# l13039968960/stm32H7-YOLO

Measured on AMD Instinct MI355X. Metric: images/sec int8 YOLO-face 56x56, higher is better.
Workload: dtype int8; 1 GPU; BASELINE configs[1]: batch=4096 int8 YOLO-face 56x56x3 frames per GPU, fused LDS-resident forward + GPU box decode; frames_per_gpu=4096, global_batch=4096, frame_bytes_in=9408, frame_bytes_out=882, input_batches_rotated=8, input_bytes_resident=308281344, kernel=yoloface56_fused<F=2,NW=8>, requant_rounding=ref, parallelism=single GPU, gather_every=1, collectives_issued=0, launch_streams=2

## Files before the change

### stm32h7-yolo_amd/csrc/yf_fused56.hip.h

```cpp


template <class B, int C, int F, int NT>
__device__ __forceinline__ void dump_buf(const char* frames, int8_t* dump, long stride, long off, long first_frame,
                                         long n_frames, int tid, int ch0 = 0, int split = 1 << 30, int gap = 0) {
  if (!dump) return;
  for (int i = tid; i < F * B::P * C; i += NT) {
    const int ch = i % C; const int t = i / C;
    const int p = t % B::P; const int f = t / B::P;
    if (first_frame + f >= n_frames) continue;
    const int phys = ch0 + ch + (ch >= split ? gap : 0);
    dump[(first_frame + f) * stride + off + (long)p * C + ch] = (int8_t)frames[f * B::FS + B::at_p(p) + phys];
  }
}

template <class B, int C, int FT, int NT, class IdOf>
__device__ __forceinline__ void dump_sets(const char* frames, int8_t* dump, long stride, long off, const IdOf& id_of, int tid, int ch0 = 0, int split = 1 << 30, int gap = 0) {
  for (int i = tid; i < FT * B::P * C; i += NT) {
    const int ch = i % C; const int t = i / C;
    const int p = t % B::P; const int f = t / B::P;
    const long id = id_of(f);
    if (id < 0) continue;
    const int phys = ch0 + ch + (ch >= split ? gap : 0);
    dump[id * stride + off + (long)p * C + ch] = (int8_t)frames[f * B::FS + B::at_p(p) + phys];
  }
}

struct DumpOffsets {
  enum { T1 = 0, T2 = T1 + 6272, T3 = T2 + 6272, T4 = T3 + 3136, Q21 = T4 + 14112, T6 = Q21 + 3528, T7 = T6 + 3528,
         T8 = T7 + 1176, T9 = T8 + 7056, T11 = T9 + 7056, T14 = T11 + 1176, T15 = T14 + 7056, Q45 = T15 + 4704,
         T17 = Q45 + 1176, T18 = T17 + 1176, T19 = T18 + 392, T20 = T19 + 1960, T22 = T20 + 1960, T23 = T22 + 392,
         T24 = T23 + 1960, T26 = T24 + 1960, T30 = T26 + 392, T31 = T30 + 2352, T32 = T31 + 1960, T33 = T32 + 1960,
         P8 = T33 + 1568, C17 = P8 + 3528, P25 = C17 + 1176, C34 = P25 + 1176, C40 = C34 + 392, L43 = C40 + 392,
         TOTAL = L43 + 1176 };
};

struct NetParams {
  const int8_t* in;
  int8_t* out;
  long n;
  const uint8_t* tab;
  int8_t* dump;
  int stop_stage;
  yf_det* dets;
  int* counts;
  int cap, mode;
  int q_thr;
  float w_scale, h_scale;
  char* scratch;
};
static_assert(sizeof(yf_table_index) <= YF_INDEX_RESERVED, "index does not fit its reserved slot");
typedef const __attribute__((address_space(4))) char* kargs_ptr;
__device__ __forceinline__ kargs_ptr kargs_here() {
  kargs_ptr p = (kargs_ptr)__builtin_amdgcn_kernarg_segment_ptr();
  asm volatile("" : "+s"(p));
  return p;
}
#define YF_ARG(FIELD) (*reinterpret_cast<const __attribute__((address_space(4))) decltype(NetParams::FIELD)*>(kargs_here() + offsetof(NetParams, FIELD)))

#ifndef YF_POOL_MERGE
#define YF_POOL_MERGE 1
#endif
#ifndef YF_POOL8H_WAVES
#define YF_POOL8H_WAVES 3
#endif
#ifndef YF_POOL8V_WAVES
#define YF_POOL8V_WAVES 3
#endif
#ifndef YF_PRIO_LIST
#define YF_PRIO_LIST 3,3,3,3,3,3,3,3,3,3, 2,2,2,2, 1,1,1,1,1,1, 0,0,0,0,0,0,0
#endif
constexpr int STAGE_PRIO[27] = {YF_PRIO_LIST};
template <int K> __device__ __forceinline__ void stage_prio() {
  if constexpr (K == 0 || STAGE_PRIO[K] != STAGE_PRIO[K - 1]) __builtin_amdgcn_s_setprio(STAGE_PRIO[K]);
}
#if defined(YF_LAB) && defined(YF_DUMP_PROD_ORDER)
#define YF_PDUMP 1
#else
#define YF_PDUMP 0
#endif
template <bool DUMP> constexpr bool tail_batch() { return !DUMP || YF_PDUMP; }

template <int F, int NW, bool DUMP, bool CAM = false>
#if !defined(YF_LAB) || !defined(YF_TPJ13)
#undef YF_TPJ13
#define YF_TPJ13 3
#endif
#if !defined(YF_LAB) || !defined(YF_TPJ23)
#undef YF_TPJ23
#define YF_TPJ23 2
#endif
#if defined(YF_LAB) && defined(YF_WHATIF_WPE)
#define YF_WPE(NW) YF_WHATIF_WPE
#else
#define YF_WPE(NW) ((NW) == 12 ? 6 : (NW) >= 8 ? 4 : ((NW) == 6 ? 3 : 2))
#endif
__global__ void __launch_bounds__(NW * 64, YF_WPE(NW)) yoloface56_fused(const NetParams prm) {
  extern __shared__ __attribute__((aligned(16))) char smem[];
  constexpr int NT = NW * 64;
  constexpr bool BATCH = tail_batch<DUMP>();
  constexpr bool POOL_MERGE = YF_POOL_MERGE != 0 && (!DUMP || YF_PDUMP) && NW >= 8;
  constexpr bool XDUMP = DUMP && !YF_PDUMP;
  typedef Buf<B_T14::OFF, 14, 14, 32, 14, 0, 0> B_T6X;
  typedef typename std::conditional<POOL_MERGE, B_T6X, B_T6>::type B_T6M;
  constexpr int FT = BATCH ? 2 * F : F;
  typedef TailBufs<BATCH ? FRAME_STRIDE / 2 : FRAME_STRIDE> U;
  constexpr int OUT_ALL_BYTES = BATCH ? 0 : (F * OUT_FRAME_BYTES + 15) & ~15;
  static_assert(std::is_same<decltype(&yoloface56_fused<F, NW, DUMP, CAM>), void (*)(const NetParams)>::value, "YF_ARG: NetParams is the kernel's only argument (kernarg offset 0)");
  uint8_t* luts = reinterpret_cast<uint8_t*>(smem);
  constexpr int PRE = v2::pre_bytes<F, tail_batch<DUMP>()>();
  char* out_all = smem + PRE;
  char* frames = smem + PRE + OUT_ALL_BYTES;
  const int n_frames = (int)prm.n;
  const int tid0 = threadIdx.x;
  const uint8_t* __restrict__ tab = prm.tab;
  int vz = 0;
  asm volatile("" : "+v"(vz));
  const __attribute__((address_space(1))) uint8_t* lut_src = (const __attribute__((address_space(1))) uint8_t*)(tab + PLAN.lut_off);
  asm volatile("" : "+s"(lut_src));
  for (int i = tid0; i < v2::LUT_B / 16; i += NT)
    reinterpret_cast<v4u*>(luts)[i] = *(const __attribute__((address_space(1))) v4u*)(lut_src + (uint32_t)(16 * i));
  for (int i = tid0; i < v2::ZERO_B / 16; i += NT) reinterpret_cast<uint4*>(smem + v2::ZERO)[i] = uint4{0, 0, 0, 0};
  constexpr int DBG_LUT = PRE + OUT_ALL_BYTES + FRAME_BYTES + (F - 1) * FRAME_STRIDE;
  if constexpr (DUMP) { if (tid0 < YF_DBG_LUT_BYTES / 16) reinterpret_cast<v4u*>(smem + DBG_LUT)[tid0] = *(const __attribute__((address_space(1))) v4u*)(lut_src + (uint32_t)(YF_N_LUT * 256 + YF_ADDLUT_BYTES + 16 * tid0)); }
#if !(defined(YF_LAB) && defined(YF_WHATIF_NO_PROLOGUE_TABLES))
  {
    typedef v2::JobTabs<F, tail_batch<DUMP>()> JTS;
    typedef typename JTS::U UT;
    v2::fill_jobtab<F, 1, B_T1, B_T2, JTS::JT_DW3>(smem, tid0);
    v2::fill_jobtab<F, 2, B_T4, B_T6M, JTS::JT_DW10>(smem, tid0);
    v2::fill_jobtab<F, 1, B_T8, B_T9, JTS::JT_DW15>(smem, tid0);
    v2::fill_jobtab<JTS::FT, 2, typename UT::T15, typename UT::T17, JTS::JT_DW27>(smem, tid0);
    v2::fill_jobtab<JTS::FT, 1, typename UT::T19, typename UT::T20, JTS::JT_DW32>(smem, tid0);
    typedef v2::HaloTabs<F, tail_batch<DUMP>()> HTS;
    v2::build_halotab<typename HTS::G1, HTS::H_T1, NT>(smem, tid0);
    v2::build_halotab<typename HTS::G4, HTS::H_T4, NT>(smem, tid0);
    v2::build_halotab<typename HTS::G8, HTS::H_T8, NT>(smem, tid0);
    v2::build_halotab<typename HTS::G15, HTS::H_T15, NT>(smem, tid0);
    v2::build_halotab<typename HTS::G19, HTS::H_T19, NT>(smem, tid0);
  }
#endif

  auto sfresh = [](int v) { asm volatile("" : "+s"(v)); return v; };
  auto n_groups = [&]() { return (int)((uint32_t)(sfresh(n_frames) + F - 1) / (uint32_t)F); };
  int gstep = (int)gridDim.x;
  asm volatile("" : "+s"(gstep));
  auto park_slot = [&]() { return YF_ARG(scratch) + (uint32_t)(sfresh((int)blockIdx.x) * (F * TailBufs<FRAME_BYTES>::T15_BYTES)); };
  const AddK no_add = {};
  auto addctx = [&](int k) {
    const uint8_t* a = tab + offsetof(yf_table_index, add) + k * sizeof(yf_add);
    return AddK{uniform_u32(a + offsetof(yf_add, mo2)), uniform_u32(a + offsetof(yf_add, zro)),
                (unsigned long)uniform_u32(a + offsetof(yf_add, c64o)) | ((unsigned long)uniform_u32(a + offsetof(yf_add, c64o) + 4) << 32),
                (int)uniform_u32(a + offsetof(yf_add, rso))};
  };
  constexpr long DS = DumpOffsets::TOTAL;
#ifdef YF_BARPROF
  bool prof_on = false;
  int bar_no = 0;
  long long* prof_out = reinterpret_cast<long long*>(prm.dump) + ((long)blockIdx.x * NW + __builtin_amdgcn_readfirstlane(tid0 >> 6)) * 80;
#define YF_SYNC() do { asm volatile("s_waitcnt vmcnt(0)" ::: "memory");    \
                       if (prof_on && (tid0 & 63) == 0 && bar_no < 40) prof_out[2 * bar_no] = __builtin_readcyclecounter(); __syncthreads(); \
                       if (prof_on && (tid0 & 63) == 0 && bar_no < 40) prof_out[2 * bar_no + 1] = __builtin_readcyclecounter(); ++bar_no; } while (0)
#else
#define YF_SYNC() do { asm volatile("s_waitcnt vmcnt(0)" ::: "memory"); __syncthreads(); } while (0)
#endif
#define YF_HALO(B, RING, FR, G, HOFF, WI, TID) \
  do { int ht_ = TID; asm volatile("" : "+v"(ht_)); \
       v2::fill_halo_t<B, typename v2::HaloTabs<F, BATCH>::G, v2::HaloTabs<F, BATCH>::HOFF>(frames, load_halo_zp(tab, WI), ht_); } while (0)
#define YF_FETCH(CS, WV, LN) v2::fetch_consts_s<CS>(tab, WV, LN)
#define YF_CONV1(WV, LN, CS) v2::conv1_2_stage<F, NW, CS>(frames, tab, WV, LN)
#define YF_DENSE(FR, TPJ, KS, BW, IN, OUT, CH0, COUT, EPI, LUT, ADDB, DI, AD, WV, LN, CS) \
  v2::dense2_stage<FR, NW, TPJ, KS, BW, IN, OUT, CH0, COUT, EPI, LUT, ADDB, CS>(frames, out_all, tab, AD, WV, LN)
#define YF_DW(FR, STRIDE, IN, OUT, C, LUT, WI, WV, LN, CS, JTOFF) v2::dw2_stage<FR, NW, STRIDE, IN, OUT, C, LUT, CS, v2::JobTabs<F, BATCH>::JTOFF>(frames, tab, WV, LN)
#define YF_DUMP(BUF, C, OFF, ...) \
  if constexpr (DUMP) { if (prm.dump) { dump_buf<BUF, C, F, NT>(frames, prm.dump, DS, DumpOffsets::OFF, first, n_frames, tid, ##__VA_ARGS__); YF_SYNC(); } }
  int stage_no = 0;
#define YF_STAGE_END() if constexpr (DUMP) { if (++stage_no == prm.stop_stage) continue; }
#define YF_PRIO(K) stage_prio<K>()

  int prev_first = -1;
  auto decode_prev = [&](int w, int ln) {
    if (prm.dets != nullptr && prev_first >= 0 && w >= NW - F && prev_first + (w - (NW - F)) < n_frames) {
      int dl = ln;
      asm volatile("" : "+v"(dl));
      yfdec::decode_frame(reinterpret_cast<const int8_t*>(out_all) + (w - (NW - F)) * OUT_FRAME_BYTES, prev_first + (w - (NW - F)), dl,
                          prm.mode, prm.w_scale, prm.h_scale, prm.dets, prm.counts, prm.cap);
// ... 325 lines not shown
```

### stm32h7-yolo_amd/csrc/yf_kernels.hip.h

```cpp
#include <hip/hip_runtime.h>
#include <stddef.h>
#include <stdint.h>
#include <type_traits>
#include "yf_tables.h"

#pragma clang diagnostic push
#pragma clang diagnostic ignored "-Wint-to-pointer-cast"
#if !defined(YF_LAB) || !defined(YF_LAUNDER)
#undef YF_LAUNDER
#define YF_LAUNDER 0
#endif
#define YF_ROW_SKEW 4
#define YF_T8_ROW_SKEW 32
namespace YF_NS {

#ifndef YF_NOINLINE_STAGES
#define YF_STAGE_FN __device__ __forceinline__
#else
#define YF_STAGE_FN __device__ __attribute__((noinline))
#endif

typedef int v4i __attribute__((ext_vector_type(4)));
typedef short v2s __attribute__((ext_vector_type(2)));

#if !defined(YF_H0) || YF_H0 == 56
constexpr int FRAME_BYTES = 34176;
#endif
constexpr int LUT_BYTES = YF_N_LUT * 256 + YF_ADDLUT_BYTES;


#if !defined(YF_H0) || YF_H0 == 56
#if defined(YF_LAB) && defined(YF_WHATIF_FS)
constexpr int FRAME_STRIDE = YF_WHATIF_FS;
#else
constexpr int FRAME_STRIDE = FRAME_BYTES;
#endif
constexpr int BUF_FS = FRAME_STRIDE;
#else
constexpr int BUF_FS = 0;
#endif
template <int OFF_, int W_, int H_, int S_, int RS_, int PT_, int PL_, int FS_ = BUF_FS, int SK_ = 0>
struct Buf {
  static constexpr int OFF = OFF_, W = W_, H = H_, S = S_, RS = RS_, PT = PT_, PL = PL_, FS = FS_, SK = SK_;
  static constexpr int P = W_ * H_, ROWB = RS_ * S_ + SK_;
  __device__ static __forceinline__ int at(int y, int x) { return OFF_ + (y + PT_) * ROWB + (x + PL_) * S_; }
  __device__ static __forceinline__ int at_p(int p) {
    if constexpr (RS_ == W_ && PT_ == 0 && PL_ == 0) return OFF_ + p * S_;
    else { const int y = p / W_; return at(y, p - y * W_); }
  }
};
template <int WIDTH>
constexpr bool lds_conflict_free(const int (&addr)[32]) {
  for (int i = 0; i < 32; ++i) {
    if (addr[i] % WIDTH != 0) return false;
    for (int j = 0; j < i; ++j)
      if (addr[i] != addr[j] && (addr[i] / WIDTH) % 32 == (addr[j] / WIDTH) % 32) return false;
  }
  return true;
}

#ifndef YF_H0
#define YF_H0 56
#endif
constexpr int G0 = YF_H0, G1 = G0 / 2, G2 = G0 / 4, G3 = G0 / 8;
static_assert(G0 % 8 == 0 && G3 >= 4, "input size must be a multiple of 8 and at least 32");

#if YF_H0 == 56
typedef Buf<    0, 56, 56,  4, 60, 1, 4> B_IN;
typedef Buf<13696, 28, 28,  8, 30, 1, 1, BUF_FS, YF_ROW_SKEW> B_T1;
typedef Buf<21024, 28, 28,  8, 28, 0, 0> B_T2;
typedef Buf<16832, 28, 28,  4, 28, 0, 0> B_T3;
typedef Buf<    0, 28, 28, 20, 29, 1, 1> B_T4;
typedef Buf<16832, 14, 28, 20, 14, 0, 0> B_HB;
typedef Buf<24672, 14, 14, 48, 14, 0, 0> B_T14;
typedef Buf<16832, 14, 14, 32, 14, 0, 0> B_T6;
typedef Buf<    0, 14, 14,  8, 14, 0, 0> B_T7;
typedef Buf< 1568, 14, 14, 36, 16, 1, 1, BUF_FS, YF_T8_ROW_SKEW> B_T8;
typedef Buf<11296, 14, 14, 48, 14, 0, 0> B_T9;
typedef Buf<20704, 14, 14,  8, 14, 0, 0> B_T11;
typedef Buf<    0, 14, 14, 24, 15, 1, 1> B_T15;
typedef Buf< 5408,  7,  7, 48,  7, 0, 0> B_T30;
typedef Buf< 7760,  7,  7, 32,  7, 0, 0> B_T17;
typedef Buf< 9328,  7,  7,  8,  7, 0, 0> B_T18;
typedef Buf< 9728,  7,  7, 40,  9, 1, 1, BUF_FS, YF_ROW_SKEW> B_T19;
typedef Buf<13008,  7,  7, 48,  7, 0, 0> B_T20;
typedef Buf<15360,  7,  7,  8,  7, 0, 0> B_T22;
typedef Buf<15752,  7,  7,  8,  7, 0, 0> B_T26;
typedef Buf<16144,  7,  7, 32,  7, 0, 0> B_T33;
template <int FS_>
struct TailBufs {
  typedef Buf<    0, 14, 14, 24, 15, 1, 1, FS_> T15;
  typedef Buf< 5408,  7,  7, 48,  7, 0, 0, FS_> T30;
  typedef Buf< 7760,  7,  7, 32,  7, 0, 0, FS_> T17;
  typedef Buf< 9328,  7,  7,  8,  7, 0, 0, FS_> T18;
  typedef Buf< 9728,  7,  7, 40,  9, 1, 1, FS_, YF_ROW_SKEW> T19;
  typedef Buf<13008,  7,  7, 48,  7, 0, 0, FS_> T20;
  typedef Buf<15360,  7,  7,  8,  7, 0, 0, FS_> T22;
  typedef Buf<15752,  7,  7,  8,  7, 0, 0, FS_> T26;
  typedef Buf< 7760,  7,  7, 32,  7, 0, 0, FS_> T33;
  typedef Buf<16160,  7,  7, 18,  7, 0, 0, FS_> HEAD;
  static constexpr int END = 16160 + 882, T15_BYTES = 5408;
  static_assert(T19::OFF + 9 * T19::ROWB <= T20::OFF && T20::OFF + 49 * 48 <= T22::OFF && T26::OFF + 49 * 8 <= HEAD::OFF, "tail buffers do not overlap");
#if !(defined(YF_LAB) && defined(YF_WHATIF_FS))
  static_assert(END <= FS_, "a set fits its stride");
#endif
};
#else
constexpr int arena_next(int off, int bytes) { return (off + bytes + 64 + 63) & ~63; }
#define YF_SEQ(NAME, PREV_END, W_, H_, S_, RS_, PT_, PL_, ROWS_)                      \
  constexpr int NAME##_OFF = PREV_END;                                                \
  typedef Buf<NAME##_OFF, W_, H_, S_, RS_, PT_, PL_> NAME;                            \
  constexpr int NAME##_END = arena_next(NAME##_OFF, (ROWS_) * (RS_) * (S_));
YF_SEQ(B_IN,  0,         G0, G0,  4, G0 + 4, 1, 4, G0 + 1)
YF_SEQ(B_T1,  B_IN_END,  G1, G1,  8, G1 + 2, 1, 1, G1 + 2)
YF_SEQ(B_T2,  B_T1_END,  G1, G1,  8, G1,     0, 0, G1)
YF_SEQ(B_T3,  B_T2_END,  G1, G1,  4, G1,     0, 0, G1)
YF_SEQ(B_T4,  B_T3_END,  G1, G1, 20, G1 + 1, 1, 1, G1 + 1)
YF_SEQ(B_HB,  B_T4_END,  G2, G1, 20, G2,     0, 0, G1)
YF_SEQ(B_T14, B_HB_END,  G2, G2, 48, G2,     0, 0, G2)
YF_SEQ(B_T6,  B_T14_END, G2, G2, 32, G2,     0, 0, G2)
YF_SEQ(B_T7,  B_T6_END,  G2, G2,  8, G2,     0, 0, G2)
YF_SEQ(B_T8,  B_T7_END,  G2, G2, 36, G2 + 2, 1, 1, G2 + 2)
YF_SEQ(B_T9,  B_T8_END,  G2, G2, 48, G2,     0, 0, G2)
YF_SEQ(B_T11, B_T9_END,  G2, G2,  8, G2,     0, 0, G2)
YF_SEQ(B_T15, B_T11_END, G2, G2, 24, G2 + 1, 1, 1, G2 + 1)
YF_SEQ(B_T30, B_T15_END, G3, G3, 48, G3,     0, 0, G3)
YF_SEQ(B_T17, B_T30_END, G3, G3, 32, G3,     0, 0, G3)
YF_SEQ(B_T18, B_T17_END, G3, G3,  8, G3,     0, 0, G3)
YF_SEQ(B_T19, B_T18_END, G3, G3, 40, G3 + 2, 1, 1, G3 + 2)
YF_SEQ(B_T20, B_T19_END, G3, G3, 48, G3,     0, 0, G3)
YF_SEQ(B_T22, B_T20_END, G3, G3,  8, G3,     0, 0, G3)
YF_SEQ(B_T26, B_T22_END, G3, G3,  8, G3,     0, 0, G3)
YF_SEQ(B_T33, B_T26_END, G3, G3, 32, G3,     0, 0, G3)
#undef YF_SEQ
#endif

#if YF_H0 != 56
constexpr int FRAME_BYTES = B_T33_END;
#endif
constexpr int OUT_FRAME_BYTES = G3 * G3 * 18;
constexpr int IN_FRAME_BYTES = G0 * G0 * 3;

enum { EPI_LUT = 0, EPI_RAW = 1, EPI_ADD = 2, EPI_HEAD = 3, EPI_HEAD_LDS = 4 };

typedef unsigned v4u __attribute__((ext_vector_type(4)));
typedef unsigned v2u __attribute__((ext_vector_type(2)));
typedef unsigned long v4ul __attribute__((ext_vector_type(4)));
template <bool AFTER_MFMA, bool SIGNLESS = false>
__device__ __forceinline__ void rq4(const v4i acc, const v4u m2, const v4u zr, const v4ul c64, int (&t)[4]) {
  v2u d0, d1, d2, d3;
  if constexpr (SIGNLESS) {
    (void)zr;
#define YF_RQ3_MADS "v_mad_u64_u32 %0, vcc, %4, %8, %12\n\tv_mad_u64_u32 %1, vcc, %5, %9, %13\n\t" \
                    "v_mad_u64_u32 %2, vcc, %6, %10, %14\n\tv_mad_u64_u32 %3, vcc, %7, %11, %15"
#define YF_RQ3_OPS : "=&v"(d0), "=&v"(d1), "=&v"(d2), "=&v"(d3) \
                   : "v"(acc[0]), "v"(acc[1]), "v"(acc[2]), "v"(acc[3]), "v"(m2[0]), "v"(m2[1]), "v"(m2[2]), "v"(m2[3]), \
                     "s"(c64[0]), "s"(c64[1]), "s"(c64[2]), "s"(c64[3]) : "vcc"
    if constexpr (AFTER_MFMA) asm("s_nop 7\n\ts_nop 1\n\t" YF_RQ3_MADS YF_RQ3_OPS);
    else asm(YF_RQ3_MADS YF_RQ3_OPS);
#undef YF_RQ3_MADS
#undef YF_RQ3_OPS
    t[0] = (int)d0[1]; t[1] = (int)d1[1]; t[2] = (int)d2[1]; t[3] = (int)d3[1];
    return;
  }
  unsigned long cy0, cy1, cy2, cy3;
#define YF_RQ4_MADS "v_mad_u64_u32 %0, %4, %8, %12, %16\n\tv_mad_u64_u32 %1, %5, %9, %13, %17\n\t" \
                    "v_mad_u64_u32 %2, %6, %10, %14, %18\n\tv_mad_u64_u32 %3, %7, %11, %15, %19"
#define YF_RQ4_OPS : "=&v"(d0), "=&v"(d1), "=&v"(d2), "=&v"(d3), "=&s"(cy0), "=&s"(cy1), "=&s"(cy2), "=&s"(cy3) \
                   : "v"(acc[0]), "v"(acc[1]), "v"(acc[2]), "v"(acc[3]), "v"(m2[0]), "v"(m2[1]), "v"(m2[2]), "v"(m2[3]), \
                     "s"(c64[0]), "s"(c64[1]), "s"(c64[2]), "s"(c64[3])
  if constexpr (AFTER_MFMA) asm("s_nop 7\n\ts_nop 1\n\t" YF_RQ4_MADS YF_RQ4_OPS);
  else asm(YF_RQ4_MADS YF_RQ4_OPS);
#undef YF_RQ4_MADS
#undef YF_RQ4_OPS
  asm("v_addc_co_u32_e64 %0, vcc, %4, %8, %12\n\tv_addc_co_u32_e64 %1, vcc, %5, %9, %13\n\t"
      "v_addc_co_u32_e64 %2, vcc, %6, %10, %14\n\tv_addc_co_u32_e64 %3, vcc, %7, %11, %15"
      : "=&v"(t[0]), "=&v"(t[1]), "=&v"(t[2]), "=&v"(t[3])
      : "v"(zr[0]), "v"(zr[1]), "v"(zr[2]), "v"(zr[3]), "v"(d0[1]), "v"(d1[1]), "v"(d2[1]), "v"(d3[1]),
        "s"(cy0), "s"(cy1), "s"(cy2), "s"(cy3)
      : "vcc");
}
__device__ __forceinline__ int rqf(int acc, uint32_t fs, int k) {
  const float p = (float)acc * __uint_as_float(fs);
  return min(max(__float_as_int(p + 0x1.8p23f) - k, 0), 255);
}
// ... 449 lines not shown
  }
}

template <int W, int SH = (W > 32 ? 20 : 16)> struct DivW {
  static constexpr uint32_t M = ((1u << SH) + W - 1) / W;
  static constexpr bool ok() { for (uint32_t p = 0; p < 2048; ++p) if (((p * M) >> SH) != p / W) return false; return true; }
  static_assert(ok(), "multiply-shift division is exact on [0, 2048)");
  __device__ static __forceinline__ int div(int p) { return (int)(((uint32_t)p * M) >> SH); }
};

template <int EPI, int LUT_ID, int LA, int STASH_LUT = -1>
__device__ __forceinline__ void epilogue2(char* dstpix, const char* addpix, char* headpix, int chq, int hq, const int (&idx)[4], const AddK& ad,
                                          char* stashpix = nullptr) {
  if constexpr (EPI == EPI_LUT) {
    *reinterpret_cast<uint32_t*>(dstpix + chq) = join4(lutb<LUT_ID>(idx[0]), lutb<LUT_ID>(idx[1]), lutb<LUT_ID>(idx[2]), lutb<LUT_ID>(idx[3]));
    if constexpr (STASH_LUT >= 0) {
      if (stashpix) *reinterpret_cast<uint32_t*>(stashpix + chq) =
          join4(*(lds_u8_ptr)(uint32_t)(STASH_LUT + idx[0]), *(lds_u8_ptr)(uint32_t)(STASH_LUT + idx[1]),
                *(lds_u8_ptr)(uint32_t)(STASH_LUT + idx[2]), *(lds_u8_ptr)(uint32_t)(STASH_LUT + idx[3]));
    }
  } else if constexpr (EPI == EPI_RAW) {
    *reinterpret_cast<uint32_t*>(dstpix + chq) = join4(idx[0], idx[1], idx[2], idx[3]) ^ 0x80808080u;
  } else if constexpr (EPI == EPI_ADD) {
    typedef const __attribute__((address_space(3))) int* lds_i32_ptr;
    if (stashpix) *reinterpret_cast<uint32_t*>(stashpix + chq) = join4(idx[0], idx[1], idx[2], idx[3]) ^ 0x80808080u;
    const uint32_t o = lds_u32(addpix + chq) ^ 0x80808080u;
    v4i sum;
#pragma unroll
    for (int j = 0; j < 4; ++j)
      sum[j] = *(lds_i32_ptr)(uint32_t)(LA + 4 * ((o >> (8 * j)) & 255)) + *(lds_i32_ptr)(uint32_t)(LA + 1024 + 4 * idx[j]);
    int r[4];
    requant4<false>(sum, v4u{ad.mo2, ad.mo2, ad.mo2, ad.mo2}, v4u{ad.zro, ad.zro, ad.zro, ad.zro},
                    v4ul{ad.c64o, ad.c64o, ad.c64o, ad.c64o}, v4i{ad.rso, ad.rso, ad.rso, ad.rso}, r);
    *reinterpret_cast<uint32_t*>(dstpix + chq) = join4(r[0], r[1], r[2], r[3]) ^ 0x80808080u;
  } else {
    const uint32_t v = join4(idx[0], idx[1], idx[2], idx[3]) ^ 0x80808080u;
    uint16_t* dst = reinterpret_cast<uint16_t*>(headpix + hq);
    dst[0] = (uint16_t)v;
    if (hq + 2 < 18) dst[1] = (uint16_t)(v >> 16);
  }
}

template <int EPI, int LUT_ID, int LA>
__device__ __forceinline__ void epilogue2_half(char* dstpix, const char* addpix, int chq, const int (&idx)[2], const AddK& ad) {
  static_assert(EPI == EPI_LUT || EPI == EPI_RAW || EPI == EPI_ADD, "half passes: LUT, raw and residual-add epilogues");
  if constexpr (EPI == EPI_LUT) {
    *reinterpret_cast<uint32_t*>(dstpix + chq) = join2(lutb<LUT_ID>(idx[0]), lutb<LUT_ID>(idx[1]));
  } else if constexpr (EPI == EPI_RAW) {
    *reinterpret_cast<uint32_t*>(dstpix + chq) = join2(idx[0], idx[1]) ^ 0x8080u;
  } else {
    typedef const __attribute__((address_space(3))) int* lds_i32_ptr;
    const uint32_t o = lds_u32(addpix + chq) ^ 0x80808080u;
    v4i sum = {0, 0, 0, 0};
#pragma unroll
    for (int j = 0; j < 2; ++j)
      sum[j] = *(lds_i32_ptr)(uint32_t)(LA + 4 * ((o >> (8 * j)) & 255)) + *(lds_i32_ptr)(uint32_t)(LA + 1024 + 4 * idx[j]);
    int r[2];
    requant2<false>(sum, v4u{ad.mo2, ad.mo2, ad.mo2, ad.mo2}, v4u{ad.zro, ad.zro, ad.zro, ad.zro},
                    v4ul{ad.c64o, ad.c64o, ad.c64o, ad.c64o}, v4i{ad.rso, ad.rso, ad.rso, ad.rso}, r);
    *reinterpret_cast<uint32_t*>(dstpix + chq) = join2(r[0], r[1]) ^ 0x8080u;
  }
}
#if !defined(YF_LAB) || !defined(YF_CHUNK_UNROLL)
#undef YF_CHUNK_UNROLL
#define YF_CHUNK_UNROLL 0
#endif
#define YF_HALF_PASS 1

template <int F, int NW, int TPJ, int KS, int BW, class IN, class OUT, int OUT_CH0, int COUT, int EPI, int LUT_ID, class ADDB, int CS,
          int STASH_OFF = -1, int STASH_S = 0, int STASH_LUT = -1, class LAY = Lay56, int LA_ABS = -1>
YF_STAGE_FN void dense2_stage(char* frames, char* out_all, const uint8_t* __restrict__ tab, const AddK ad, int wave, int lane) {
  constexpr int NP = (COUT + 3) / 4, NCH = (NP + TPJ - 1) / TPJ;
  constexpr int P = IN::P, TOT = F * P;
  constexpr bool FRAME_TILES = P <= 64;
  constexpr int MT = FRAME_TILES ? F : (TOT + 63) / 64;
  constexpr int JOBS = NCH * MT, KROW = 16 * KS;
  constexpr int SLOT = LAY::slot(CS), WB = plan_wbytes(CS), PV = SLOT + WB, LA = LA_ABS >= 0 ? LA_ABS : PV + NP * (int)sizeof(yf_pass_v);
  static_assert(yf_cs_dense[CS] >= 0 && KROW == PLAN_KROW[yf_cs_dense[CS]] && NP == plan_passes(CS), "stage and constant block agree");
  static_assert((EPI == EPI_ADD) == (yf_cs_add[CS] >= 0), "residual-add tables travel with their stage");
  static_assert(OUT::P == P || EPI == EPI_HEAD || EPI == EPI_HEAD_LDS, "1x1 conv keeps the grid");
  static_assert(IN::FS == OUT::FS && IN::FS == ADDB::FS, "one frame stride per stage");
  static_assert(IN::S >= 16 * (KS - 1) + BW && (BW == 4 || BW == 8 || BW == 16), "the pixel vector must cover all k-steps");
  static_assert(IN::RS == IN::W && IN::PT == 0 && IN::PL == 0, "dense inputs are plain buffers");
  const int g = lane >> 4, c = lane & 15;
  const bool a_on = (c >> 2) == g;
  const uint32_t a_lane = a_on ? (uint32_t)(SLOT + (c & 3) * KROW) : (uint32_t)LAY::ZERO;
  const uint32_t a_step = a_on ? (uint32_t)(TPJ * 4 * KROW) : 0u;
  const uint8_t* sc = tab + PLAN.sb_off[CS];
  int in_c = 0, out_c = 0, add_c = 0, stash_c = 0;
  static_assert(STASH_OFF < 0 || EPI == EPI_ADD || (EPI == EPI_LUT && STASH_LUT >= 0), "a stash is the pre-add convolution output or a second LUT's view");
  if constexpr (FRAME_TILES) {
    const int p = min(lane, P - 1);
    in_c = IN::OFF + p * IN::S;
    if constexpr (EPI == EPI_HEAD || EPI == EPI_HEAD_LDS) out_c = p * 18;
    else if constexpr (OUT::RS == OUT::W && OUT::PT == 0 && OUT::PL == 0) out_c = OUT::OFF + p * OUT::S + OUT_CH0;
    else { const int y = DivW<OUT::W>::div(p); out_c = OUT::at(y, p - y * OUT::W) + OUT_CH0; }
    add_c = ADDB::OFF + p * ADDB::S;
    if constexpr (STASH_OFF >= 0) stash_c = STASH_OFF + p * STASH_S;
  }
  int j0, j1;
  job_range<JOBS, NW>(wave, j0, j1);
  auto run_chunk = [&](const int chunk, int mt, const int n) __attribute__((always_inline)) {
    v4i a[TPJ][KS];
    PassV pv[TPJ];
    PassS ksr[TPJ];
    const uint32_t a_addr = a_lane + (uint32_t)chunk * a_step;
#pragma unroll
    for (int t = 0; t < TPJ; ++t) {
      const int ps = chunk * TPJ + t;
#pragma unroll
      for (int ks = 0; ks < KS; ++ks) a[t][ks] = lds_v4i(a_addr + (uint32_t)(t * 4 * KROW + 16 * ks));
      pv[t].m2 = lds_v4u((uint32_t)(PV + ps * 32));
      pv[t].zr = lds_v4u((uint32_t)(PV + ps * 32 + 16));
      const uint8_t* s = sc + min(ps, NP - 1) * (int)sizeof(yf_pass_s);
      ksr[t] = PassS{*(cv4ul_ptr)(uintptr_t)s, *(cv4i_ptr)(uintptr_t)(s + 32)};
    }
    const int cq = chunk * TPJ * 4;
    const int out_cc = out_c + cq, add_cc = add_c + cq;
    for (int k = 0; k < n; ++k, ++mt) {
      const char* src; char* dstpix = nullptr; const char* addpix = nullptr; char* headpix = nullptr; char* stashpix = nullptr;
      if constexpr (FRAME_TILES) {
        char* fbase = frames + mt * IN::FS;
        src = fbase + in_c;
        dstpix = fbase + out_cc; addpix = fbase + add_cc;
        if constexpr (STASH_OFF >= 0) stashpix = fbase + stash_c + cq;
        if constexpr (EPI == EPI_HEAD) headpix = out_all + mt * OUT_FRAME_BYTES + out_c;
        if constexpr (EPI == EPI_HEAD_LDS) headpix = fbase + OUT::OFF + out_c;
      } else {
        const int q = min(mt * 64 + lane, TOT - 1);
        int f = 0;
#pragma unroll
        for (int i = 1; i < F; ++i) f += (q >= i * P) ? 1 : 0;
        const int p = q - f * P;
        char* fbase = frames + f * IN::FS;
        src = fbase + IN::OFF + p * IN::S;
        if constexpr (EPI == EPI_HEAD) headpix = out_all + f * OUT_FRAME_BYTES + p * 18;
        else if constexpr (EPI == EPI_HEAD_LDS) headpix = fbase + OUT::OFF + p * 18;
        else if constexpr (OUT::RS == OUT::W && OUT::PT == 0 && OUT::PL == 0) dstpix = fbase + cq + OUT::OFF + p * OUT::S + OUT_CH0;
        else { const int y = DivW<OUT::W>::div(p); dstpix = fbase + cq + OUT::at(y, p - y * OUT::W) + OUT_CH0; }
        if constexpr (EPI == EPI_ADD) addpix = fbase + cq + ADDB::OFF + p * ADDB::S;
        if constexpr (STASH_OFF >= 0) stashpix = fbase + cq + STASH_OFF + p * STASH_S;
      }
      v4i b[KS];
#pragma unroll
      for (int ks = 0; ks < KS - 1; ++ks) b[ks] = *reinterpret_cast<const v4i*>(src + 16 * ks);
      const char* last = src + 16 * (KS - 1);
      if constexpr (BW == 16) b[KS - 1] = *reinterpret_cast<const v4i*>(last);
      else if constexpr (BW == 8) { const int2 t2 = *reinterpret_cast<const int2*>(last); b[KS - 1] = v4i{t2.x, t2.y, any_value(), any_value()}; }
      else b[KS - 1] = v4i{*reinterpret_cast<const int*>(last), any_value(), any_value(), any_value()};
#pragma unroll
      for (int t = 0; t < TPJ; ++t) {
        const int ps = chunk * TPJ + t;
        if (ps < NP) {
          v4i acc = acc_init(pv[t].zr);
#pragma unroll
          for (int ks = 0; ks < KS; ++ks) acc = __builtin_amdgcn_mfma_i32_16x16x64_i8(a[t][ks], b[ks], acc, 0, 0, 0);
          constexpr bool HALF_L = YF_HALF_PASS && COUT % 4 == 2 && STASH_OFF < 0 && (EPI == EPI_LUT || EPI == EPI_RAW || EPI == EPI_ADD);
          const bool half = HALF_L && t == (NP - 1) % TPJ && ps == NP - 1;
          if (half) {
            if constexpr (HALF_L) {
              int idx2[2];
              requant2<true, DENSE_SIGNLESS, RQ_FP32>(acc, pv[t].m2, pv[t].zr, ksr[t].c64, ksr[t].rs, idx2);
              epilogue2_half<EPI, LUT_ID, LA>(dstpix, addpix, t * 4, idx2, ad);
            }
          } else {
            int idx[4];
            requant4<true, DENSE_SIGNLESS, RQ_FP32>(acc, pv[t].m2, pv[t].zr, ksr[t].c64, ksr[t].rs, idx);
            epilogue2<EPI, LUT_ID, LA, STASH_LUT>(dstpix, addpix, headpix, t * 4, ps * 4, idx, ad, stashpix);
          }
        }
      }
    }
  };
  if constexpr (NCH <= YF_CHUNK_UNROLL) {
#pragma unroll
    for (int chunk = 0; chunk < NCH; ++chunk) {
      const int lo = max(j0, chunk * MT), hi = min(j1, (chunk + 1) * MT);
      if (lo < hi) run_chunk(chunk, lo - chunk * MT, hi - lo);
    }
  } else {
    int chunk = (int)((uint32_t)j0 / (uint32_t)MT), mt = j0 - chunk * MT, left = j1 - j0;
    while (left > 0) {
      const int n = min(left, MT - mt);
      run_chunk(chunk, mt, n);
      left -= n; ++chunk; mt = 0;
    }
  }
}

template <int F, class IN, class OUT>
constexpr bool conv1_pairs_conflict_free(int arena0) {
  if (IN::RS % 2 != 0) return false;
  for (int q0 = 0; q0 < F * OUT::P; q0 += 32) {
    int addr[32] = {};
    for (int l = 0; l < 32; ++l) {
      const int q = q0 + l < F * OUT::P ? q0 + l : F * OUT::P - 1, f = q / OUT::P, p = q - f * OUT::P, oy = p / OUT::W, ox = p - oy * OUT::W;
      addr[l] = arena0 + f * IN::FS + IN::OFF + 4 * (2 * oy * IN::RS + 2 * ox + 4);
    }
    if (!lds_conflict_free<8>(addr)) return false;
  }
  return true;
}
template <int F, int NW, int CS, class IN = B_IN, class OUT = B_T1, class LAY = Lay56>
YF_STAGE_FN void conv1_2_stage(char* frames, const uint8_t* __restrict__ tab, int wave, int lane) {
  constexpr int P = OUT::P, W1 = OUT::W, RSW = IN::RS, TOT = F * P;
  constexpr int MT = (TOT + 63) / 64;
  constexpr int SLOT = LAY::slot(CS), WB = plan_wbytes(CS), PV = SLOT + WB;
  const int g = lane >> 4, c = lane & 15;
  const bool a_on = (c >> 2) == g;
  const uint32_t a_addr = a_on ? (uint32_t)(SLOT + (c & 3) * YF_CONV1_KROW) : (uint32_t)LAY::ZERO;
  const uint8_t* sc = tab + PLAN.sb_off[CS];
  static_assert(RSW % 2 == 0 && IN::OFF % 8 == 0 && IN::FS % 8 == 0, "the tap pairs (kx = 1, 2) of a kernel row are 8-byte aligned");
  v4i a[2][3];
  PassV pv[2];
#pragma unroll
  for (int ps = 0; ps < 2; ++ps) {
    v4i t[3];
#pragma unroll
    for (int ks = 0; ks < 3; ++ks) t[ks] = lds_v4i(a_addr + (uint32_t)(ps * 4 * YF_CONV1_KROW + 16 * ks));
    a[ps][0] = v4i{t[0][0], t[0][3], t[0][1], t[0][2]};
    a[ps][1] = v4i{t[1][0], t[1][1], t[1][3], t[2][0]};
    a[ps][2] = v4i{t[1][2], t[2][1], t[2][2], t[2][3]};
    pv[ps].m2 = lds_v4u((uint32_t)(PV + ps * 32));
    pv[ps].zr = lds_v4u((uint32_t)(PV + ps * 32 + 16));
  }
  int j0, j1;
  job_range<MT, NW>(wave, j0, j1);
  const AddK ad = {};
  for (int mt = j0; mt < j1; ++mt) {
    const int q = min(mt * 64 + lane, TOT - 1);
    int f = 0;
#pragma unroll
    for (int i = 1; i < F; ++i) f += (q >= i * P) ? 1 : 0;
    const int p = q - f * P;
    const int oy = DivW<W1>::div(p), ox = p - oy * W1;
    char* fbase = frames + f * IN::FS;
    const uint32_t* src = reinterpret_cast<const uint32_t*>(fbase + IN::OFF) + (2 * oy * RSW + 2 * ox + 3);
    const uint2 r0 = *reinterpret_cast<const uint2*>(src + 1), r1 = *reinterpret_cast<const uint2*>(src + RSW + 1), r2 = *reinterpret_cast<const uint2*>(src + 2 * RSW + 1);
    const v4i b0 = {(int)src[0], (int)src[RSW], (int)r0.x, (int)r0.y};
    const v4i b1 = {(int)r1.x, (int)r1.y, (int)r2.x, (int)r2.y};
    const v4i b2 = {(int)src[2 * RSW], any_value(), any_value(), any_value()};
    char* dstpix = fbase + OUT::at(oy, ox);
#pragma unroll
    for (int ps = 0; ps < 2; ++ps) {
      const uint8_t* s = sc + ps * (int)sizeof(yf_pass_s);
      const PassS k = PassS{*(cv4ul_ptr)(uintptr_t)s, *(cv4i_ptr)(uintptr_t)(s + 32)};
      v4i acc = acc_init(pv[ps].zr);
      acc = __builtin_amdgcn_mfma_i32_16x16x64_i8(a[ps][0], b0, acc, 0, 0, 0);
      acc = __builtin_amdgcn_mfma_i32_16x16x64_i8(a[ps][1], b1, acc, 0, 0, 0);
      acc = __builtin_amdgcn_mfma_i32_16x16x64_i8(a[ps][2], b2, acc, 0, 0, 0);
      int idx[4];
      requant4<true, DENSE_SIGNLESS, RQ_FP32>(acc, pv[ps].m2, pv[ps].zr, k.c64, k.rs, idx);
      epilogue2<EPI_LUT, YF_L_LEAKY2, 0>(dstpix, nullptr, nullptr, 4 * ps, 0, idx, ad);
    }
  }
}

struct DwWalk { int R, FG; };
template <int F, int STRIDE, int W, int H>
constexpr DwWalk dw_rows_per_lane() {
#if YF_H0 == 56
  if (STRIDE == 1 && F == 2 && W == 28 && H == 28) return DwWalk{7, 1};
  if (STRIDE == 1 && F == 2 && W == 14 && H == 14) return DwWalk{2, 1};
  if (STRIDE == 2 && F == 2 && W == 14 && H == 14) return DwWalk{7, 2};
  if (STRIDE == 2 && F == 4 && W == 7 && H == 7) return DwWalk{4, 2};
#endif
  return DwWalk{1, 1};
}
template <int F, int STRIDE, class IN, class OUT>
struct DwGeo {
  static constexpr int W = OUT::W, H = OUT::H;
  static constexpr DwWalk WK = dw_rows_per_lane<F, STRIDE, OUT::W, OUT::H>();
  static constexpr int R = WK.R, FG = WK.FG, RG = 4 / FG, BR = RG * R;
  static constexpr int FL = (W <= 8 && F % 2 == 0) ? 2 : 1;
  static constexpr int NSEG = (W + 15) / 16, NRB = (H + BR - 1) / BR, NFP = F / (FL * FG);
  static constexpr int JPG = NFP * NRB * NSEG;
  static_assert(OUT::RS == W && OUT::PT == 0 && OUT::PL == 0, "depthwise outputs are plain buffers");
  static_assert(IN::FS == OUT::FS, "one frame stride per stage");
  static_assert((H >= BR || (R > 1 && H >= R)) && (W >= 16 || W * FL <= 16) && F % (FL * FG) == 0 && RG * FG == 4, "tile shape");
  static constexpr int seg_row_c(int rs) { return BR > H && rs * R > H - R ? H - R : rs * R; }
  __device__ static __forceinline__ int seg_row(int rs) { return BR > H ? min(rs * R, H - R) : rs * R; }
  static constexpr bool taps_conflict_free() {
    for (int half = 0; half < 2; ++half) {
      int addr[32] = {};
      for (int l = 0; l < 32; ++l) {
        const int g = 2 * half + l / 16, c = l % 16;
        const int fl = FL == 2 ? c / 8 : 0, xc = FL == 2 ? c % 8 : c, xl = xc < W - 1 ? xc : W - 1;
        addr[l] = (fl + FL * (g / RG)) * IN::FS + seg_row_c(g % RG) * STRIDE * IN::ROWB + xl * STRIDE * IN::S;
      }
      if (!lds_conflict_free<4>(addr)) return false;
    }
    return true;
  }
  __device__ static __forceinline__ uint2 job(int jj) {
    const int fp = jj / (NRB * NSEG); int rem = jj - fp * (NRB * NSEG);
    const int rb = rem / NSEG, seg = rem - rb * NSEG;
    const int oy0 = BR > H ? 0 : min(rb * BR, H - BR);
    const int x0 = (W >= 16) ? min(seg * 16, W - 16) : 0;
    const int fb = fp * FL * FG * IN::FS;
    return uint2{(uint32_t)(fb + IN::OFF + (oy0 * STRIDE) * IN::ROWB + x0 * STRIDE * IN::S), (uint32_t)(fb + OUT::OFF + (oy0 * W + x0) * OUT::S)};
  }
};
#if YF_H0 == 56
template <int F, bool BATCH>
struct JobTabs {
  typedef TailBufs<BATCH ? FRAME_STRIDE / 2 : FRAME_STRIDE> U;
  static constexpr int FT = BATCH ? 2 * F : F;
  static constexpr int JT_DW3 = 0;
  static constexpr int JT_DW10 = JT_DW3 + 8 * DwGeo<F, 1, B_T1, B_T2>::JPG;
  static constexpr int JT_DW15 = JT_DW10 + 8 * DwGeo<F, 2, B_T4, B_T6>::JPG;
  static constexpr int JT_DW27 = JT_DW15 + 8 * DwGeo<F, 1, B_T8, B_T9>::JPG;
  static constexpr int JT_DW32 = JT_DW27 + 8 * DwGeo<FT, 2, typename U::T15, typename U::T17>::JPG;
  static constexpr int END = JT_DW32 + 8 * DwGeo<FT, 1, typename U::T19, typename U::T20>::JPG;
  static_assert(END <= JT_B, "job tables fit");
};
#endif
template <class B, bool RING, int F>
struct HaloGeo {
  static constexpr int HR = B::H + B::PT + (RING ? 1 : 0), WR = B::RS;
  static constexpr int NPIX = RING ? (2 * WR + 2 * (HR - 2)) : (WR + HR - 1);
  static constexpr int N = F * NPIX;
  static_assert(B::S % 4 == 0 && B::OFF % 4 == 0 && B::FS % 4 == 0, "dword pixels");
  __device__ static __forceinline__ uint32_t entry(int i) {
    const int f = i / NPIX, k = i - f * NPIX;
    int r, c;
    if constexpr (RING) {
      if (k < WR) { r = 0; c = k; }
      else if (k < 2 * WR) { r = HR - 1; c = k - WR; }
      else { const int m = k - 2 * WR; r = 1 + (m >> 1); c = (m & 1) ? WR - 1 : 0; }
    } else {
      if (k < WR) { r = 0; c = k; } else { r = 1 + (k - WR); c = 0; }
    }
    return (uint32_t)(f * B::FS + B::OFF + r * B::ROWB + c * B::S);
  }
};
#if YF_H0 == 56
template <int F, bool BATCH>
struct HaloTabs {
  typedef TailBufs<BATCH ? FRAME_STRIDE / 2 : FRAME_STRIDE> U;
  static constexpr int FT = BATCH ? 2 * F : F;
  typedef HaloGeo<B_T1, true, F> G1; typedef HaloGeo<B_T4, false, F> G4; typedef HaloGeo<B_T8, true, F> G8;
  typedef HaloGeo<B_T15, false, F> G15; typedef HaloGeo<typename U::T19, true, FT> G19;
  static constexpr int H_T1 = 0, H_T4 = H_T1 + 2 * G1::N, H_T8 = H_T4 + 2 * G4::N, H_T15 = H_T8 + 2 * G8::N, H_T19 = H_T15 + 2 * G15::N;
  static constexpr int BYTES = (H_T19 + 2 * G19::N + 15) & ~15;
};
constexpr int HT = SLOT0 + 2 * SLOT_B;
template <int F, bool BATCH> constexpr int pre_bytes() { return HT + HaloTabs<F, BATCH>::BYTES; }
#if !(defined(YF_LAB) && defined(YF_WHATIF_FS))
static_assert(DwGeo<2, 1, B_T1, B_T2>::taps_conflict_free(), "conv2d_3: the tap reads of a half-wave fall on distinct LDS banks");
static_assert(DwGeo<2, 1, B_T8, B_T9>::taps_conflict_free(), "conv2d_15: the tap reads of a half-wave fall on distinct LDS banks");
static_assert(conv1_pairs_conflict_free<2, B_IN, B_T1>(pre_bytes<2, true>()) && conv1_pairs_conflict_free<2, B_IN, B_T1>(pre_bytes<2, false>()) &&
              conv1_pairs_conflict_free<1, B_IN, B_T1>(pre_bytes<1, true>()) && conv1_pairs_conflict_free<1, B_IN, B_T1>(pre_bytes<1, false>()),
              "conv2d_1: the tap pairs of a half-wave fall on distinct LDS bank pairs");
static_assert(pool8_rows_conflict_free<2>(pre_bytes<2, true>()) && pool8_rows_conflict_free<2>(pre_bytes<2, false>()),
              "pool_8 h (rows across the lanes): every read of the sweep puts the rows of a half-wave on distinct LDS banks");
#endif
static_assert(B_T7::OFF + B_T7::P * B_T7::S <= B_T8::OFF && B_T8::OFF + (B_T8::H + 2) * B_T8::ROWB <= B_T9::OFF && B_T9::OFF + B_T9::P * B_T9::S <= B_T11::OFF &&
              B_T11::OFF + B_T11::P * B_T11::S <= B_T14::OFF, "T7 | T8 | T9 | T11 | concat_22 do not overlap");
template <class G, int HOFF, int NT>
__device__ __forceinline__ void build_halotab(char* smem, int tid) {
  for (int i = tid; i < G::N; i += NT) *reinterpret_cast<uint16_t*>(smem + HT + HOFF + 2 * i) = (uint16_t)(G::entry(i) >> 2);
}
template <class B, class G, int HOFF>
YF_STAGE_FN void fill_halo_t(char* frames, int zp, int tid) {
  typedef const __attribute__((address_space(3))) uint16_t* lds_u16_ptr;
  if (tid < G::N) {
    const uint32_t v = (uint32_t)(zp & 255) * 0x01010101u;
    char* p = frames + 4u * (uint32_t)*(lds_u16_ptr)(uint32_t)(HT + HOFF + 2 * tid);
    if constexpr (B::S % 8 == 0 && B::OFF % 8 == 0 && B::FS % 8 == 0) {
#pragma unroll
      for (int d = 0; d < B::S / 8; ++d) *reinterpret_cast<uint2*>(p + 8 * d) = uint2{v, v};
    } else {
#pragma unroll
      for (int d = 0; d < B::S / 4; ++d) *reinterpret_cast<uint32_t*>(p + 4 * d) = v;
    }
  }
}
#endif

template <int F, int STRIDE, class IN, class OUT, int JTOFF, class LAY = Lay56>
__device__ __forceinline__ void fill_jobtab(char* smem, int tid) {
  typedef DwGeo<F, STRIDE, IN, OUT> G;
  static_assert(JTOFF % 8 == 0 && JTOFF + G::JPG * 8 <= LAY::JT_BYTES, "job table in bounds");
  if (tid < G::JPG) *reinterpret_cast<uint2*>(smem + LAY::JT + JTOFF + 8 * tid) = G::job(tid);
}

template <int F, int NW, int STRIDE, class IN, class OUT, int C, int LUT_ID, int CS, int JTOFF, class LAY = Lay56>
YF_STAGE_FN void dw2_stage(char* frames, const uint8_t* __restrict__ tab, int wave, int lane) {
  typedef DwGeo<F, STRIDE, IN, OUT> G;
  constexpr int W = G::W, FL = G::FL, JPG = G::JPG;
  constexpr int NG = (C + 3) / 4, JOBS = NG * JPG;
  constexpr int DROW = STRIDE * IN::ROWB;
  constexpr int TS = IN::S, TR = IN::ROWB;
  constexpr int SLOT = LAY::slot(CS);
  static_assert(yf_cs_dw[CS] >= 0 && NG == plan_passes(CS), "stage and constant block agree");
  const int g = lane >> 4, c = lane & 15;
  const int fl = (FL == 2) ? (c >> 3) : 0;
  const int xl = (FL == 2) ? min(c & 7, W - 1) : min(c, W - 1);
  const int fr = fl + FL * (g / G::RG), row0 = G::seg_row(g % G::RG);
  const char* lane_in = frames + fr * IN::FS + row0 * DROW + xl * STRIDE * IN::S;
  char* lane_out = frames + fr * IN::FS + (row0 * W + xl) * OUT::S;
  const bool a_on = (c >> 2) == g;
  const uint32_t a_lane = a_on ? (uint32_t)(SLOT + 4 * (c & 3)) : (uint32_t)LAY::ZERO;
  const uint32_t a_step = a_on ? (uint32_t)YF_DWV_GROUP_BYTES : 0u;
  const uint8_t* sc = tab + PLAN.sb_off[CS];
  int j, j1;
  job_range<JOBS, NW>(wave, j, j1);
  int cg = (int)((uint32_t)j / (uint32_t)JPG), jj = j - cg * JPG, left = j1 - j;
  while (left > 0) {
    const uint32_t wa = a_lane + (uint32_t)cg * a_step;
    v4i a0, a1, a2 = {0, 0, 0, 0};
    a0 = v4i{(int)*(lds_u32_ptr)(wa), (int)*(lds_u32_ptr)(wa + 16), (int)*(lds_u32_ptr)(wa + 32), (int)*(lds_u32_ptr)(wa + 48)};
    a1 = v4i{(int)*(lds_u32_ptr)(wa + 64), (int)*(lds_u32_ptr)(wa + 80), (int)*(lds_u32_ptr)(wa + 96), (int)*(lds_u32_ptr)(wa + 112)};
    a2[0] = (int)*(lds_u32_ptr)(wa + 128);
    PassV pv;
    pv.m2 = lds_v4u((uint32_t)(SLOT + cg * YF_DWV_GROUP_BYTES + 144));
    pv.zr = lds_v4u((uint32_t)(SLOT + cg * YF_DWV_GROUP_BYTES + 160));
    const uint8_t* s = sc + cg * (int)sizeof(yf_pass_s);
    const PassS k = PassS{*(cv4ul_ptr)(uintptr_t)s, *(cv4i_ptr)(uintptr_t)(s + 32)};
    const char* lin = lane_in + 4 * cg;
    char* lout = lane_out + 4 * cg;
    auto entry = [&](int job) { return *(lds_u2_ptr)(uint32_t)(LAY::JT + JTOFF + 8 * min(job, JPG - 1)); };
    auto taps = [&](const v2u e, v4i& b0, v4i& b1, v4i& b2, char*& dst) {
      const char* src = lin + e[0];
      b0[0] = (int)lds_u32(src);               b0[1] = (int)lds_u32(src + TS);          b0[2] = (int)lds_u32(src + 2 * TS);
      b0[3] = (int)lds_u32(src + TR);          b1[0] = (int)lds_u32(src + TR + TS);     b1[1] = (int)lds_u32(src + TR + 2 * TS);
      b1[2] = (int)lds_u32(src + 2 * TR);      b1[3] = (int)lds_u32(src + 2 * TR + TS); b2[0] = (int)lds_u32(src + 2 * TR + 2 * TS);
      dst = lout + e[1];
    };
    auto conv = [&](const v4i& b0, const v4i& b1, const v4i& b2) {
      v4i acc = acc_init(pv.zr);
      acc = __builtin_amdgcn_mfma_i32_16x16x64_i8(a0, b0, acc, 0, 0, 0);
      acc = __builtin_amdgcn_mfma_i32_16x16x64_i8(a1, b1, acc, 0, 0, 0);
      return __builtin_amdgcn_mfma_i32_16x16x64_i8(a2, b2, acc, 0, 0, 0);
    };
    auto finish = [&](const v4i& acc, char* dst) {
      if (YF_HALF_PASS && C % 4 == 2 && cg == NG - 1) {
        int idx2[2];
// ... 98 lines not shown
```

Before: 33.09 million images/s.

## Pad T6/T17/T33 channel strides to 48 bytes and pair dense LUT stores

Widens the per-pixel stride of the 32-channel buffers T6 (merged-pool variant), T17 and T33 to 48 bytes and relocates T17/T33 into freed slots (T20's and T19's regions), so the ds_read_b128 loads of the following dense convs avoid LDS bank conflicts. It also adds a paired-store path in the dense stage that combines two adjacent pixels' requantized dwords into a single 8-byte store. Compile-time checks for bank ways and buffer overlap guard the new layout. The cost is a larger buffer footprint inside the frame, which depends on the liveness assumptions about the reused slots being correct.

```diff
diff --git a/stm32h7-yolo_amd/csrc/yf_fused56.hip.h b/stm32h7-yolo_amd/csrc/yf_fused56.hip.h
--- a/stm32h7-yolo_amd/csrc/yf_fused56.hip.h
+++ b/stm32h7-yolo_amd/csrc/yf_fused56.hip.h
@@ -100,7 +100,10 @@
   constexpr bool BATCH = tail_batch<DUMP>();
   constexpr bool POOL_MERGE = YF_POOL_MERGE != 0 && (!DUMP || YF_PDUMP) && NW >= 8;
   constexpr bool XDUMP = DUMP && !YF_PDUMP;
-  typedef Buf<B_T14::OFF, 14, 14, 32, 14, 0, 0> B_T6X;
+  typedef Buf<B_T14::OFF, 14, 14, 48, 14, 0, 0> B_T6X;
+  static_assert(B_T6X::OFF + B_T6X::P * B_T6X::S <= B_T14::OFF + B_T14::P * B_T14::S && B_T14::OFF + B_T14::P * B_T14::S <= FRAME_BYTES, "T6 stays inside concat_22's region");
+  static_assert(dense_b128_conflicts<1, B_T6X>() == 0 && dense_b128_conflicts<2, B_T6X>() <= 1, "conv2d_12: the ds_read_b128 of T6 are free of bank conflicts inside a frame");
+  static_assert(v2::DwGeo<2, 2, B_T4, B_T6X>::store_ways() <= 4, "conv2d_10: the stores into T6 are at most 4-way");
   typedef typename std::conditional<POOL_MERGE, B_T6X, B_T6>::type B_T6M;
   constexpr int FT = BATCH ? 2 * F : F;
   typedef TailBufs<BATCH ? FRAME_STRIDE / 2 : FRAME_STRIDE> U;
diff --git a/stm32h7-yolo_amd/csrc/yf_kernels.hip.h b/stm32h7-yolo_amd/csrc/yf_kernels.hip.h
--- a/stm32h7-yolo_amd/csrc/yf_kernels.hip.h
+++ b/stm32h7-yolo_amd/csrc/yf_kernels.hip.h
@@ -57,6 +57,63 @@
       if (addr[i] != addr[j] && (addr[i] / WIDTH) % 32 == (addr[j] / WIDTH) % 32) return false;
   }
   return true;
+}
+template <int WIDTH, int N>
+constexpr int lds_ways(const int (&addr)[N], int banks) {
+  bool first[N] = {};
+  for (int i = 0; i < N; ++i) {
+    first[i] = true;
+    for (int j = 0; j < i; ++j) if (addr[j] == addr[i]) first[i] = false;
+  }
+  int worst = 0;
+  for (int i = 0; i < N; ++i) {
+    if (!first[i]) continue;
+    int k = 0;
+    for (int j = 0; j < N; ++j) if (first[j] && (addr[j] / WIDTH) % banks == (addr[i] / WIDTH) % banks) ++k;
+    worst = k > worst ? k : worst;
+  }
+  return worst;
+}
+template <int F, class B>
+constexpr void dense_job_addrs(int mt, int (&addr)[64]) {
+  static_assert(B::RS == B::W && B::PT == 0 && B::PL == 0, "plain buffers");
+  for (int l = 0; l < 64; ++l) {
+    int f = mt, p = l < B::P ? l : B::P - 1;
+    if (B::P > 64) { const int q = mt * 64 + l < F * B::P ? mt * 64 + l : F * B::P - 1; f = q / B::P; p = q - f * B::P; }
+    addr[l] = f * B::FS + B::OFF + p * B::S;
+  }
+}
+template <int F, class B> constexpr int dense_jobs() { return B::P <= 64 ? F : (F * B::P + 63) / 64; }
+constexpr int B128_GROUP[4][16] = {{0, 1, 2, 3, 12, 13, 14, 15, 20, 21, 22, 23, 24, 25, 26, 27}, {4, 5, 6, 7, 8, 9, 10, 11, 16, 17, 18, 19, 28, 29, 30, 31},
+                                   {32, 33, 34, 35, 44, 45, 46, 47, 52, 53, 54, 55, 56, 57, 58, 59}, {36, 37, 38, 39, 40, 41, 42, 43, 48, 49, 50, 51, 60, 61, 62, 63}};
+template <int F, class IN>
+constexpr int dense_b128_conflicts() {
+  int total = 0;
+  for (int mt = 0; mt < dense_jobs<F, IN>(); ++mt) {
+    int addr[64] = {};
+    dense_job_addrs<F, IN>(mt, addr);
+    for (int g = 0; g < 4; ++g) {
+      int a16[16] = {};
+      for (int l = 0; l < 16; ++l) a16[l] = addr[B128_GROUP[g][l]];
+      total += lds_ways<16>(a16, 16) - 1;
+    }
+  }
+  return total;
+}
+template <int F, class OUT>
+constexpr int dense_pair_store_ways() {
+  int worst = 0;
+  for (int mt = 0; mt < dense_jobs<F, OUT>(); ++mt) {
+    int addr[64] = {};
+    dense_job_addrs<F, OUT>(mt, addr);
+    for (int g = 0; g < 4; ++g) {
+      int dw[32] = {};
+      for (int l = 0; l < 16; ++l) { dw[2 * l] = addr[16 * g + l]; dw[2 * l + 1] = addr[16 * g + l] + 4; }
+      const int k = lds_ways<4>(dw, 32);
+      worst = k > worst ? k : worst;
+    }
+  }
+  return worst;
 }
 
 #ifndef YF_H0
@@ -80,27 +137,31 @@
 typedef Buf<20704, 14, 14,  8, 14, 0, 0> B_T11;
 typedef Buf<    0, 14, 14, 24, 15, 1, 1> B_T15;
 typedef Buf< 5408,  7,  7, 48,  7, 0, 0> B_T30;
-typedef Buf< 7760,  7,  7, 32,  7, 0, 0> B_T17;
+typedef Buf<13008,  7,  7, 48,  7, 0, 0> B_T17;
 typedef Buf< 9328,  7,  7,  8,  7, 0, 0> B_T18;
 typedef Buf< 9728,  7,  7, 40,  9, 1, 1, BUF_FS, YF_ROW_SKEW> B_T19;
 typedef Buf<13008,  7,  7, 48,  7, 0, 0> B_T20;
 typedef Buf<15360,  7,  7,  8,  7, 0, 0> B_T22;
 typedef Buf<15752,  7,  7,  8,  7, 0, 0> B_T26;
-typedef Buf<16144,  7,  7, 32,  7, 0, 0> B_T33;
+typedef Buf< 9728,  7,  7, 48,  7, 0, 0> B_T33;
 template <int FS_>
 struct TailBufs {
   typedef Buf<    0, 14, 14, 24, 15, 1, 1, FS_> T15;
   typedef Buf< 5408,  7,  7, 48,  7, 0, 0, FS_> T30;
-  typedef Buf< 7760,  7,  7, 32,  7, 0, 0, FS_> T17;
+  typedef Buf<13008,  7,  7, 48,  7, 0, 0, FS_> T17;
   typedef Buf< 9328,  7,  7,  8,  7, 0, 0, FS_> T18;
   typedef Buf< 9728,  7,  7, 40,  9, 1, 1, FS_, YF_ROW_SKEW> T19;
   typedef Buf<13008,  7,  7, 48,  7, 0, 0, FS_> T20;
   typedef Buf<15360,  7,  7,  8,  7, 0, 0, FS_> T22;
   typedef Buf<15752,  7,  7,  8,  7, 0, 0, FS_> T26;
-  typedef Buf< 7760,  7,  7, 32,  7, 0, 0, FS_> T33;
+  typedef Buf< 9728,  7,  7, 48,  7, 0, 0, FS_> T33;
   typedef Buf<16160,  7,  7, 18,  7, 0, 0, FS_> HEAD;
   static constexpr int END = 16160 + 882, T15_BYTES = 5408;
   static_assert(T19::OFF + 9 * T19::ROWB <= T20::OFF && T20::OFF + 49 * 48 <= T22::OFF && T26::OFF + 49 * 8 <= HEAD::OFF, "tail buffers do not overlap");
+  static_assert(T17::OFF == T20::OFF && T17::P * T17::S == T20::P * T20::S && T15::OFF + T15_BYTES <= T30::OFF && T30::OFF + T30::P * T30::S <= T18::OFF &&
+                T18::OFF + T18::P * T18::S <= T17::OFF && T17::OFF + T17::P * T17::S <= T22::OFF, "T17 fills T20's slot, clear of T15, concat_46 and T18");
+  static_assert(T33::OFF == T19::OFF && T33::OFF >= 2048 && T33::OFF + T33::P * T33::S <= T19::OFF + 9 * T19::ROWB && T19::OFF + 9 * T19::ROWB <= T20::OFF &&
+                T20::OFF + T20::P * T20::S <= HEAD::OFF, "T33 lies inside T19's slot, clear of T20, the head and the decode tables");
 #if !(defined(YF_LAB) && defined(YF_WHATIF_FS))
   static_assert(END <= FS_, "a set fits its stride");
 #endif
@@ -716,6 +777,8 @@
   static_assert(IN::FS == OUT::FS && IN::FS == ADDB::FS, "one frame stride per stage");
   static_assert(IN::S >= 16 * (KS - 1) + BW && (BW == 4 || BW == 8 || BW == 16), "the pixel vector must cover all k-steps");
   static_assert(IN::RS == IN::W && IN::PT == 0 && IN::PL == 0, "dense inputs are plain buffers");
+  constexpr bool PAIR = std::is_same<LAY, Lay56>::value && EPI == EPI_LUT && STASH_OFF < 0 && STASH_LUT < 0 && TPJ % 2 == 0 && NP % TPJ == 0 &&
+                        OUT::FS % 8 == 0 && OUT::OFF % 8 == 0 && OUT::S % 8 == 0 && OUT::ROWB % 8 == 0 && OUT_CH0 % 8 == 0 && (TPJ * 4) % 8 == 0;
   const int g = lane >> 4, c = lane & 15;
   const bool a_on = (c >> 2) == g;
   const uint32_t a_lane = a_on ? (uint32_t)(SLOT + (c & 3) * KROW) : (uint32_t)LAY::ZERO;
@@ -782,9 +845,20 @@
       if constexpr (BW == 16) b[KS - 1] = *reinterpret_cast<const v4i*>(last);
       else if constexpr (BW == 8) { const int2 t2 = *reinterpret_cast<const int2*>(last); b[KS - 1] = v4i{t2.x, t2.y, any_value(), any_value()}; }
       else b[KS - 1] = v4i{*reinterpret_cast<const int*>(last), any_value(), any_value(), any_value()};
+      uint32_t even_dw = 0;
 #pragma unroll
       for (int t = 0; t < TPJ; ++t) {
         const int ps = chunk * TPJ + t;
+        if constexpr (PAIR) {
+          v4i acc = acc_init(pv[t].zr);
+#pragma unroll
+          for (int ks = 0; ks < KS; ++ks) acc = __builtin_amdgcn_mfma_i32_16x16x64_i8(a[t][ks], b[ks], acc, 0, 0, 0);
+          int idx[4];
+          requant4<true, DENSE_SIGNLESS, RQ_FP32>(acc, pv[t].m2, pv[t].zr, ksr[t].c64, ksr[t].rs, idx);
+          const uint32_t dw = join4(lutb<LUT_ID>(idx[0]), lutb<LUT_ID>(idx[1]), lutb<LUT_ID>(idx[2]), lutb<LUT_ID>(idx[3]));
+          if (t % 2 == 0) even_dw = dw;
+          else *reinterpret_cast<uint2*>(dstpix + (t - 1) * 4) = uint2{even_dw, dw};
+        } else
         if (ps < NP) {
           v4i acc = acc_init(pv[t].zr);
 #pragma unroll
@@ -926,6 +1000,20 @@
     }
     return true;
   }
+  static constexpr int store_ways() {
+    int worst = 0;
+    for (int half = 0; half < 2; ++half) {
+      int addr[32] = {};
+      for (int l = 0; l < 32; ++l) {
+        const int g = 2 * half + l / 16, c = l % 16;
+        const int fl = FL == 2 ? c / 8 : 0, xc = FL == 2 ? c % 8 : c, xl = xc < W - 1 ? xc : W - 1;
+        addr[l] = (fl + FL * (g / RG)) * OUT::FS + (seg_row_c(g % RG) * W + xl) * OUT::S;
+      }
+      const int k = lds_ways<4>(addr, 32);
+      worst = k > worst ? k : worst;
+    }
+    return worst;
+  }
   __device__ static __forceinline__ uint2 job(int jj) {
     const int fp = jj / (NRB * NSEG); int rem = jj - fp * (NRB * NSEG);
     const int rb = rem / NSEG, seg = rem - rb * NSEG;
@@ -988,6 +1076,11 @@
               "conv2d_1: the tap pairs of a half-wave fall on distinct LDS bank pairs");
 static_assert(pool8_rows_conflict_free<2>(pre_bytes<2, true>()) && pool8_rows_conflict_free<2>(pre_bytes<2, false>()),
               "pool_8 h (rows across the lanes): every read of the sweep puts the rows of a half-wave on distinct LDS banks");
+typedef TailBufs<FRAME_STRIDE / 2> TailSets;
+static_assert(dense_b128_conflicts<4, TailSets::T17>() <= dense_jobs<4, TailSets::T17>(), "conv2d_29: the ds_read_b128 of T17 are free of bank conflicts but for the surplus lanes");
+static_assert(dense_b128_conflicts<4, TailSets::T33>() <= dense_jobs<4, TailSets::T33>(), "conv2d_53: the ds_read_b128 of T33 are free of bank conflicts but for the surplus lanes");
+static_assert(DwGeo<4, 2, TailSets::T15, TailSets::T17>::store_ways() <= 4, "conv2d_27: the stores into T17 are at most 4-way");
+static_assert(dense_pair_store_ways<4, TailSets::T33>() <= 2, "conv2d_51: the paired stores into T33 are at most 2-way");
 #endif
 static_assert(B_T7::OFF + B_T7::P * B_T7::S <= B_T8::OFF && B_T8::OFF + (B_T8::H + 2) * B_T8::ROWB <= B_T9::OFF && B_T9::OFF + B_T9::P * B_T9::S <= B_T11::OFF &&
               B_T11::OFF + B_T11::P * B_T11::S <= B_T14::OFF, "T7 | T8 | T9 | T11 | concat_22 do not overlap");
```

Result: no change. 33.38 million images/s, median of 6 (+0.9%).
